# JanLohse/raw2film

Measured on AMD Instinct MI355X. Metric: megapixels/sec full film pipeline (neg+print+grain+halation+MTF), 100MP frame, higher is better.
Workload: dtype f32 (pointwise stages, grain) + f64 (FFT stencils; the MTF's scratch images are complex64)

## Files before the change

raw2film_amd/csrc/r2f_front.hip:

```cpp
#include <algorithm>
#include <type_traits>

#include "r2f_launch.h"

#include "../../include/r2f.h"

#ifndef R2F_FRONT_LUT_BATCH
#define R2F_FRONT_LUT_BATCH 4
#endif

namespace r2f {

namespace {

struct V3 {
    float2v xy;
    float z;
};

__device__ __forceinline__ float2v splat(float v) { return (float2v){v, v}; }

__device__ __forceinline__ V3 texel(const void* base, unsigned off) {
    const float4 t = *reinterpret_cast<const float4*>(static_cast<const char*>(base) + off);
    return V3{(float2v){t.x, t.y}, t.z};
}

__device__ __forceinline__ uint32_t u8_of(float v) {
    return (uint32_t)__builtin_amdgcn_fmed3f(v * 255.0f, 0.0f, 255.0f);
}

struct Mat3Pairs {
    float2v c0, c1, c2;
    float r0, r1, r2;
};
__device__ __forceinline__ Mat3Pairs pairs_of(const Mat3& M) {
    float m[6];
#pragma unroll
    for (int i = 0; i < 6; ++i) m[i] = __uint_as_float(__builtin_amdgcn_readfirstlane(__float_as_uint(M.m[i])));
    return Mat3Pairs{(float2v){m[0], m[3]}, (float2v){m[1], m[4]}, (float2v){m[2], m[5]}, M.m[6], M.m[7], M.m[8]};
}
__device__ __forceinline__ V3 matrix3(const Mat3Pairs& M, float r, float g, float b) {
    V3 o;
    o.xy = __builtin_elementwise_fma(M.c2, splat(b), __builtin_elementwise_fma(M.c1, splat(g), M.c0 * splat(r)));
    o.z = fmaf(M.r2, b, fmaf(M.r1, g, M.r0 * r));
    return o;
}

__device__ __forceinline__ V3 texel_lds(const float4* base, unsigned off) {
    const float4 t = *reinterpret_cast<const float4*>(reinterpret_cast<const char*>(base) + off);
    return V3{(float2v){t.x, t.y}, t.z};
}

__device__ __forceinline__ V3 lut2d(const float4* tex, const int n, const V3 p) {
#pragma clang fp contract(off)
    const float S = (p.xy.x + p.xy.y) + p.z;
    const bool dark = S < 1e-12f;
    const float inv_sum = (float)(n - 1) / (dark ? 1.0f : S);
    const float2v rg = p.xy * splat(inv_sum);
    const float fr = floorf(rg.x), fg = floorf(rg.y);
    const int ri = clampi((int)fr, 0, n - 2), gi = clampi((int)fg, 0, n - 2);
    const float rf = rg.x - fr, gf = rg.y - fg;
    const float fsum = rf + gf;
    const bool lower = fsum <= 1.0f;
    const unsigned n16 = (unsigned)n << 4;
    const unsigned o0 = (unsigned)(ri * n + gi) << 4;
    const V3 rv = texel_lds(tex, o0 + n16);
    const V3 gv = texel_lds(tex, o0 + 16u);
    const V3 sv = texel_lds(tex, o0 + (lower ? 0u : n16 + 16u));
    const float wr = lower ? rf : 1.0f - gf;
    const float wg = lower ? gf : 1.0f - rf;
    const float ws = lower ? 1.0f - fsum : fsum - 1.0f;
    const float Se = dark ? 0.0f : S;
    V3 o;
    o.xy = __builtin_elementwise_fma(sv.xy, splat(ws), __builtin_elementwise_fma(gv.xy, splat(wg), rv.xy * splat(wr))) * splat(Se);
    o.z = fmaf(sv.z, ws, fmaf(gv.z, wg, rv.z * wr)) * Se;
    return o;
}

__device__ __forceinline__ void axis_nonneg(float x, float s, int n, int& lo, float& d) {
    const float t = x * s;
    const int i0 = (int)t;
    lo = min(i0, n - 2);
    d = i0 >= n - 1 ? 1.0f : fmaf(x, s, -(float)i0);
}

__device__ __forceinline__ V3 lut3d_tetra_nonneg(const float4* tex, const int n, const float s, const float r, const float g,
                                                 const float b) {
    int rl, gl, bl;
    float dr, dg, db;
    axis_nonneg(r, s, n, rl, dr);
    axis_nonneg(g, s, n, gl, dg);
    axis_nonneg(b, s, n, bl, db);
    const unsigned er = (unsigned)(n * n) << 4, eg = (unsigned)n << 4, eb = 16u;
    const unsigned o0 = (unsigned)((rl * n + gl) * n + bl) << 4;
    const bool c1 = dr >= dg, c2 = dg >= db, c3 = dr >= db, c4 = db >= dg, c5 = db >= dr;
    const unsigned e1 = c1 ? ((c2 || c3) ? er : eb) : (c4 ? eb : eg);
    const unsigned e12 = c1 ? (c2 ? er + eg : er + eb) : ((c4 || c5) ? eg + eb : eg + er);
    const float d1 = fmaxf(fmaxf(dr, dg), db), d3 = fminf(fminf(dr, dg), db), d2 = __builtin_amdgcn_fmed3f(dr, dg, db);
    const V3 c0 = texel(tex, o0);
    const V3 ca = texel(tex, o0 + e1);
    const V3 cb = texel(tex, o0 + e12);
    const V3 cz = texel(tex, o0 + (er + eg + eb));
    V3 o;
    o.xy = __builtin_elementwise_fma(splat(d3), cz.xy - cb.xy,
                                     __builtin_elementwise_fma(splat(d2), cb.xy - ca.xy, __builtin_elementwise_fma(splat(d1), ca.xy - c0.xy, c0.xy)));
    o.z = fmaf(d3, cz.z - cb.z, fmaf(d2, cb.z - ca.z, fmaf(d1, ca.z - c0.z, c0.z)));
    return o;
}

template <int LAYOUT, int UPTO, int BY, bool FIN = false>
__global__ __launch_bounds__(64 * BY) void front_fast_kernel(const FrontArgs a) {
    extern __shared__ __attribute__((aligned(16))) float4 smem4[];
    float4* lut_lds = smem4;
    float4* cells_lds = smem4 + a.lut2d.n * a.lut2d.n;
    {
        const int tid = threadIdx.y * 64 + threadIdx.x;
        const int nt = a.lut2d.n * a.lut2d.n;
        for (int i = tid; i < nt; i += 64 * BY) lut_lds[i] = a.lut2d.tex[i];
        if (UPTO >= R2F_UPTO_DENSITY || FIN) {
            const int nc = 3 * (a.curve.m - 1);
            for (int i = tid; i < nc; i += 64 * BY) cells_lds[i] = a.curve.cells[i];
        }
        __syncthreads();
    }
#ifndef R2F_FRONT_UNITS
#define R2F_FRONT_UNITS 1
#endif
    const bool track = UPTO == R2F_UPTO_EXPOSURE && a.track.blk != nullptr;
    const int W = a.W;
    const float* in = static_cast<const float*>(a.in);
    const float s3 = a.lut3d_scale * (float)(a.lut3d.n - 1);
    const long long plane = (long long)a.in_rows * W;
    const Mat3Pairs mat = pairs_of(a.mat);
    auto row_loop = [&](auto trk_tag) {
    constexpr int TRK = decltype(trk_tag)::value;
    const int groups = (a.y1 - a.y0 + BY - 1) / BY;
    constexpr bool UNITS = R2F_FRONT_UNITS && UPTO == R2F_UPTO_OUTPUT;
    const int units = groups * a.gx;
    const int g_begin = UNITS ? (int)((long long)blockIdx.x * units / gridDim.x)
                              : (TRK ? (int)((long long)blockIdx.y * groups / gridDim.y) : (int)blockIdx.y);
    const int g_end = UNITS ? (int)((long long)(blockIdx.x + 1) * units / gridDim.x)
                            : (TRK ? (int)((long long)(blockIdx.y + 1) * groups / gridDim.y) : groups);
    const int g_step = (UNITS || TRK) ? 1 : (int)gridDim.y;
    float p_lo = __builtin_inff(), p_hi = 0.f;
    int p_ty = -1, p_tx = 0;
    auto flush = [&]() {
        if (p_ty < 0) return;
        const float w_lo = wave_extreme<false>(p_lo), w_hi = wave_extreme<true>(p_hi);
        if (threadIdx.x == 63) merge_tile(a.track, p_ty << kRangeTileRowsLog2, p_tx, w_lo, w_hi);
        p_lo = __builtin_inff(), p_hi = 0.f;
    };
    for (int unit = g_begin; unit < g_end; unit += g_step) {
        const int grp = UNITS ? unit / a.gx : unit;
        const int col = UNITS ? unit - grp * a.gx : (int)blockIdx.x;
        const int x = (col * 64 + threadIdx.x) * 4;
        const int gy = a.y0 + grp * BY + threadIdx.y;
        if (gy >= a.y1) continue;
        if (TRK) {
            const int ty = gy >> kRangeTileRowsLog2;
            if (ty != p_ty || col != p_tx) {
                flush();
                p_ty = ty, p_tx = col;
            }
        }
        if (x >= W) continue;
        const long long irow = gy - a.in_gy0;
        float r[4], g[4], b[4];
        if (LAYOUT == R2F_LAYOUT_CHW) {
            const float4 v0 = *reinterpret_cast<const float4*>(in + irow * W + x);
            const float4 v1 = *reinterpret_cast<const float4*>(in + plane + irow * W + x);
            const float4 v2 = *reinterpret_cast<const float4*>(in + 2 * plane + irow * W + x);
            r[0] = v0.x, r[1] = v0.y, r[2] = v0.z, r[3] = v0.w;
            g[0] = v1.x, g[1] = v1.y, g[2] = v1.z, g[3] = v1.w;
            b[0] = v2.x, b[1] = v2.y, b[2] = v2.z, b[3] = v2.w;
        } else if (LAYOUT == R2F_LAYOUT_HWC3) {
            const float4* p4 = reinterpret_cast<const float4*>(in + (irow * W + x) * 3);
            const float4 v0 = p4[0], v1 = p4[1], v2 = p4[2];
            r[0] = v0.x, g[0] = v0.y, b[0] = v0.z;
            r[1] = v0.w, g[1] = v1.x, b[1] = v1.y;
            r[2] = v1.z, g[2] = v1.w, b[2] = v2.x;
            r[3] = v2.y, g[3] = v2.z, b[3] = v2.w;
        } else {
            const float4* p4 = reinterpret_cast<const float4*>(in + (irow * W + x) * 4);
#pragma unroll
            for (int q = 0; q < 4; ++q) {
                const float4 v = p4[q];
                r[q] = v.x, g[q] = v.y, b[q] = v.z;
            }
        }
#pragma unroll
        for (int q = 0; q < 4; ++q) {
            V3 p = a.use_matrix ? matrix3(mat, r[q], g[q], b[q]) : V3{(float2v){r[q], g[q]}, b[q]};
            p = lut2d(lut_lds, a.lut2d.n, p);
            if (UPTO == R2F_UPTO_EXPOSURE) {
                r[q] = p.xy.x, g[q] = p.xy.y, b[q] = p.z;
                if (TRK == 1) {
                    p_lo = __builtin_isunordered(r[q], g[q]) ? -__builtin_inff() : fminf(fminf(p_lo, r[q]), g[q]);
                    p_hi = fmaxf(fmaxf(p_hi, fabsf(r[q])), fabsf(g[q]));
                } else if (TRK == 2) {
                    if (a.track_mask & 1) p_lo = range_min(p_lo, r[q]), p_hi = fmaxf(p_hi, fabsf(r[q]));
                    if (a.track_mask & 2) p_lo = range_min(p_lo, g[q]), p_hi = fmaxf(p_hi, fabsf(g[q]));
                    if (a.track_mask & 4) p_lo = range_min(p_lo, b[q]), p_hi = fmaxf(p_hi, fabsf(b[q]));
                }
                if (FIN) {
                    if (a.finish_mask & 1) r[q] = curve_eval_at((const float4*)cells_lds, a.curve, 0, log10_fast(a.finish_w[0] * r[q], a.log_eps));
                    if (a.finish_mask & 2) g[q] = curve_eval_at((const float4*)cells_lds, a.curve, 1, log10_fast(a.finish_w[1] * g[q], a.log_eps));
                    if (a.finish_mask & 4) b[q] = curve_eval_at((const float4*)cells_lds, a.curve, 2, log10_fast(a.finish_w[2] * b[q], a.log_eps));
                }
                continue;
            }
            float v3[3] = {log10_fast(p.xy.x, a.log_eps), log10_fast(p.xy.y, a.log_eps), log10_fast(p.z, a.log_eps)};
            curve_eval_batch<3, 3>((const float4*)cells_lds, a.curve, 0, v3);
            if (UPTO == R2F_UPTO_DENSITY) {
                r[q] = v3[0], g[q] = v3[1], b[q] = v3[2];
                continue;
            }
            if (R2F_FRONT_LUT_BATCH > 1) {
                r[q] = v3[0], g[q] = v3[1], b[q] = v3[2];
                continue;
            }
            if (__builtin_amdgcn_ballot_w64(fminf(fminf(v3[0], v3[1]), v3[2]) < 0.0f) == 0) {
                p = lut3d_tetra_nonneg(a.lut3d.tex, a.lut3d.n, s3, v3[0], v3[1], v3[2]);
                r[q] = p.xy.x, g[q] = p.xy.y, b[q] = p.z;
            } else {
                apply_lut3d_tetra(a.lut3d, s3, v3[0], v3[1], v3[2]);
                r[q] = v3[0], g[q] = v3[1], b[q] = v3[2];
            }
        }
        if (UPTO == R2F_UPTO_OUTPUT && R2F_FRONT_LUT_BATCH > 1) {
            constexpr int NB = R2F_FRONT_LUT_BATCH > 1 ? R2F_FRONT_LUT_BATCH : 2;
#pragma unroll
            for (int q0 = 0; q0 < 4; q0 += NB) {
                float rn[NB], gn[NB], bn[NB], lo = 0.f;
#pragma unroll
                for (int k = 0; k < NB; ++k) {
                    rn[k] = r[q0 + k], gn[k] = g[q0 + k], bn[k] = b[q0 + k];
                    lo = fminf(lo, fminf(fminf(rn[k], gn[k]), bn[k]));
                }
                if (__builtin_amdgcn_ballot_w64(lo < 0.0f) == 0) {
                    apply_lut3d_tetra_nonneg_batch<NB>(a.lut3d, s3, rn, gn, bn);
                } else {
#pragma unroll
                    for (int k = 0; k < NB; ++k) apply_lut3d_tetra(a.lut3d, s3, rn[k], gn[k], bn[k]);
                }
#pragma unroll
                for (int k = 0; k < NB; ++k) r[q0 + k] = rn[k], g[q0 + k] = gn[k], b[q0 + k] = bn[k];
            }
        }
        if (UPTO != R2F_UPTO_OUTPUT) {
            float* d0 = a.dst.data + (long long)(gy - a.dst.gy0) * W + x;
            float* f0 = FIN ? a.finish_dst.data + (long long)(gy - a.finish_dst.gy0) * W + x : d0;
            const long long fs = FIN ? a.finish_dst.plane_stride : 0;
            *reinterpret_cast<float4*>((FIN && (a.finish_mask & 1)) ? f0 : d0) = make_float4(r[0], r[1], r[2], r[3]);
            *reinterpret_cast<float4*>((FIN && (a.finish_mask & 2)) ? f0 + fs : d0 + a.dst.plane_stride) = make_float4(g[0], g[1], g[2], g[3]);
            *reinterpret_cast<float4*>((FIN && (a.finish_mask & 4)) ? f0 + 2 * fs : d0 + 2 * a.dst.plane_stride) =
                make_float4(b[0], b[1], b[2], b[3]);
            continue;
        }
        const long long obase = ((long long)(gy - a.out_gy0) * W + x) * 3;
        if (a.out_f32) {
            float4* o4 = reinterpret_cast<float4*>(a.out_f32 + obase);
            o4[0] = make_float4(r[0], g[0], b[0], r[1]);
            o4[1] = make_float4(g[1], b[1], r[2], g[2]);
            o4[2] = make_float4(b[2], r[3], g[3], b[3]);
        }
        if (a.out_u8) {
            uint32_t* o32 = reinterpret_cast<uint32_t*>(a.out_u8 + obase);
            o32[0] = u8_of(r[0]) | (u8_of(g[0]) << 8) | (u8_of(b[0]) << 16) | (u8_of(r[1]) << 24);
            o32[1] = u8_of(g[1]) | (u8_of(b[1]) << 8) | (u8_of(r[2]) << 16) | (u8_of(g[2]) << 24);
            o32[2] = u8_of(b[2]) | (u8_of(r[3]) << 8) | (u8_of(g[3]) << 16) | (u8_of(b[3]) << 24);
        }
    }
    if (TRK) {
        __shared__ int wg_ty[BY], wg_tx[BY];
        __shared__ float wg_lo[BY], wg_hi[BY];
        const float w_lo = wave_extreme<false>(p_lo), w_hi = wave_extreme<true>(p_hi);
        if (threadIdx.x == 63) wg_ty[threadIdx.y] = p_ty, wg_tx[threadIdx.y] = p_tx, wg_lo[threadIdx.y] = w_lo, wg_hi[threadIdx.y] = w_hi;
        __syncthreads();
        if (threadIdx.y == 0 && threadIdx.x == 0) {
            for (int i = 0; i < BY; ++i) {
                const int ty = wg_ty[i], tx = wg_tx[i];
                if (ty < 0) continue;
                float lo = wg_lo[i], hi = wg_hi[i];
                for (int j = i + 1; j < BY; ++j)
                    if (wg_ty[j] == ty && wg_tx[j] == tx) lo = fminf(lo, wg_lo[j]), hi = fmaxf(hi, wg_hi[j]), wg_ty[j] = -1;
                merge_tile(a.track, ty << kRangeTileRowsLog2, tx, lo, hi);
            }
        }
    }
    };
    if (!track)
        row_loop(std::integral_constant<int, 0>{});
    else if (a.track_mask == 3)
        row_loop(std::integral_constant<int, 1>{});
    else
        row_loop(std::integral_constant<int, 2>{});
}

size_t fast_lds_bytes(const FrontArgs& a) {
    const size_t lut = (size_t)a.lut2d.n * a.lut2d.n * sizeof(float4);
    const size_t cells = (a.upto >= R2F_UPTO_DENSITY || a.finish_mask) ? (size_t)3 * (a.curve.m > 1 ? a.curve.m - 1 : 0) * sizeof(float4) : 0;
    return lut + cells;
}

}

bool front_fast_eligible(const FrontArgs& a) {
    if (a.out_u16) return false;
    if (!a.vec || a.lut2d.n < 2 || (long long)a.W * 16 >= (1ll << 31) || fast_lds_bytes(a) > 144 * 1024) return false;
    if ((a.upto >= R2F_UPTO_DENSITY || a.finish_mask) && !(a.curve.near && a.curve.m >= 2)) return false;
    if (a.upto == R2F_UPTO_OUTPUT && !(a.lut3d_mode == 0 && a.lut3d.n >= 2 && a.lut3d.n <= 256)) return false;
    return true;
}

template <int UPTO, int BY, bool FIN = false>
static void launch_fast(const FrontArgs& a, hipStream_t s) {
    const int quads = (a.W + 3) / 4, gx = (quads + 63) / 64;
    const int row_groups = (a.y1 - a.y0 + BY - 1) / BY;
    const size_t lds = fast_lds_bytes(a);
    const int per_cu = lds > 80 * 1024 ? 1 : (BY == 16 ? 2 : (lds > 53 * 1024 ? 2 : 3));
    int gy = per_cu * 256 / gx;
    gy = gy > row_groups ? row_groups : (gy < 1 ? 1 : gy);
    dim3 grid(gx, gy);
    const dim3 block(64, BY);
    FrontArgs b = a;
    b.gx = gx;
    if (R2F_FRONT_UNITS && UPTO == R2F_UPTO_OUTPUT) {
        const long long units = (long long)gx * row_groups;
        grid = dim3((unsigned)std::min<long long>((long long)per_cu * 256, units));
    }
    switch (a.in_layout) {
        case R2F_LAYOUT_CHW: launch_k((front_fast_kernel<R2F_LAYOUT_CHW, UPTO, BY, FIN>), grid, block, lds, s, b); break;
        case R2F_LAYOUT_HWC3: launch_k((front_fast_kernel<R2F_LAYOUT_HWC3, UPTO, BY, FIN>), grid, block, lds, s, b); break;
        default: launch_k((front_fast_kernel<R2F_LAYOUT_HWC4, UPTO, BY, FIN>), grid, block, lds, s, b); break;
    }
}

hipError_t launch_front_fast(const FrontArgs& a, hipStream_t s) {
    const bool big = fast_lds_bytes(a) > 80 * 1024;
    if (a.upto == R2F_UPTO_EXPOSURE && a.finish_mask)
        big ? launch_fast<R2F_UPTO_EXPOSURE, 16, true>(a, s) : launch_fast<R2F_UPTO_EXPOSURE, 8, true>(a, s);
    else if (a.upto == R2F_UPTO_EXPOSURE)
        big ? launch_fast<R2F_UPTO_EXPOSURE, 16>(a, s) : launch_fast<R2F_UPTO_EXPOSURE, 8>(a, s);
    else if (a.upto == R2F_UPTO_DENSITY)
        big ? launch_fast<R2F_UPTO_DENSITY, 16>(a, s) : launch_fast<R2F_UPTO_DENSITY, 8>(a, s);
    else
        big ? launch_fast<R2F_UPTO_OUTPUT, 16>(a, s) : launch_fast<R2F_UPTO_OUTPUT, 8>(a, s);
    return take_launch_status();
}

hipError_t front_fast_init_attributes() {
#define R2F_FAST_ATTR(L, U, B)                                                                                             \
    {                                                                                                                     \
        hipError_t e = hipFuncSetAttribute(reinterpret_cast<const void*>(front_fast_kernel<L, U, B>),                     \
                                           hipFuncAttributeMaxDynamicSharedMemorySize, 144 * 1024);                       \
        if (e != hipSuccess) return e;                                                                                    \
        if (U == R2F_UPTO_EXPOSURE) {                                                                                     \
            e = hipFuncSetAttribute(reinterpret_cast<const void*>(front_fast_kernel<L, U, B, true>),                      \
                                    hipFuncAttributeMaxDynamicSharedMemorySize, 144 * 1024);                              \
            if (e != hipSuccess) return e;                                                                                \
        }                                                                                                                 \
    }
#define R2F_FAST_ATTR3(U, B) R2F_FAST_ATTR(R2F_LAYOUT_HWC3, U, B) R2F_FAST_ATTR(R2F_LAYOUT_HWC4, U, B) R2F_FAST_ATTR(R2F_LAYOUT_CHW, U, B)
    R2F_FAST_ATTR3(R2F_UPTO_EXPOSURE, 8)
    R2F_FAST_ATTR3(R2F_UPTO_EXPOSURE, 16)
    R2F_FAST_ATTR3(R2F_UPTO_DENSITY, 8)
    R2F_FAST_ATTR3(R2F_UPTO_DENSITY, 16)
    R2F_FAST_ATTR3(R2F_UPTO_OUTPUT, 8)
    R2F_FAST_ATTR3(R2F_UPTO_OUTPUT, 16)
#undef R2F_FAST_ATTR3
#undef R2F_FAST_ATTR
    return hipSuccess;
}

}
```

Before: 21610.

## Software-pipeline input loads across row units in front kernel

Restructures the front-stage row loop so that the next unit's input pixels are prefetched into registers while the current unit is computed. Depending on stage, the prefetch is issued early or after the LUT work, and asm barriers keep the loads from being sunk. It also inlines a specialized finish-curve evaluation with hoisted curve constants, and clamps x to W-4 instead of skipping out-of-range lanes. It adds experiment macros (R2F_FRONT_EXP) that replace loads or computation with constants for probing, all off by default. The cost is higher register pressure, which can lower occupancy.

```diff
diff --git a/raw2film_amd/csrc/r2f_front.hip b/raw2film_amd/csrc/r2f_front.hip
--- a/raw2film_amd/csrc/r2f_front.hip
+++ b/raw2film_amd/csrc/r2f_front.hip
@@ -7,6 +7,13 @@
 
 #ifndef R2F_FRONT_LUT_BATCH
 #define R2F_FRONT_LUT_BATCH 4
+#endif
+
+#ifndef R2F_FRONT_PIPE
+#define R2F_FRONT_PIPE 7
+#endif
+#ifndef R2F_FRONT_EXP
+#define R2F_FRONT_EXP 0
 #endif
 
 namespace r2f {
@@ -63,10 +70,14 @@
     const float fsum = rf + gf;
     const bool lower = fsum <= 1.0f;
     const unsigned n16 = (unsigned)n << 4;
-    const unsigned o0 = (unsigned)(ri * n + gi) << 4;
-    const V3 rv = texel_lds(tex, o0 + n16);
-    const V3 gv = texel_lds(tex, o0 + 16u);
-    const V3 sv = texel_lds(tex, o0 + (lower ? 0u : n16 + 16u));
+    unsigned o0 = (unsigned)(ri * n + gi) << 4;
+    if (R2F_FRONT_EXP & 4) {
+        asm volatile("" ::"v"(o0));
+        o0 = 0;
+    }
+    const V3 rv = (R2F_FRONT_EXP & 4) ? V3{(float2v){0.5f, 0.4f}, 0.3f} : texel_lds(tex, o0 + n16);
+    const V3 gv = (R2F_FRONT_EXP & 4) ? V3{(float2v){0.6f, 0.3f}, 0.2f} : texel_lds(tex, o0 + 16u);
+    const V3 sv = (R2F_FRONT_EXP & 4) ? V3{(float2v){0.4f, 0.5f}, 0.4f} : texel_lds(tex, o0 + (lower ? 0u : n16 + 16u));
     const float wr = lower ? rf : 1.0f - gf;
     const float wg = lower ? gf : 1.0f - rf;
     const float ws = lower ? 1.0f - fsum : fsum - 1.0f;
@@ -150,12 +161,85 @@
         if (threadIdx.x == 63) merge_tile(a.track, p_ty << kRangeTileRowsLog2, p_tx, w_lo, w_hi);
         p_lo = __builtin_inff(), p_hi = 0.f;
     };
-    for (int unit = g_begin; unit < g_end; unit += g_step) {
+    constexpr bool PIPE = ((R2F_FRONT_PIPE) >> UPTO) & 1;
+    constexpr int NV = LAYOUT == R2F_LAYOUT_HWC4 ? 4 : 3;
+    const int wave_row = __builtin_amdgcn_readfirstlane(threadIdx.y);
+    auto locate = [&](int unit, int& col, int& gy, int& x) {
         const int grp = UNITS ? unit / a.gx : unit;
-        const int col = UNITS ? unit - grp * a.gx : (int)blockIdx.x;
-        const int x = (col * 64 + threadIdx.x) * 4;
-        const int gy = a.y0 + grp * BY + threadIdx.y;
-        if (gy >= a.y1) continue;
+        col = UNITS ? unit - grp * a.gx : (int)blockIdx.x;
+        x = min((col * 64 + (int)threadIdx.x) * 4, W - 4);
+        gy = a.y0 + grp * BY + wave_row;
+    };
+    auto fetch = [&](int gy, int x, float4(&v)[NV]) {
+        const long long irow = gy - a.in_gy0;
+        if (R2F_FRONT_EXP & 1) {
+            const float t = 0.05f + 1e-4f * (float)((x + 7 * gy) & 1023);
+#pragma unroll
+            for (int i = 0; i < NV; ++i) v[i] = make_float4(t, 2.f * t, 0.5f * t + 0.01f * i, 3.f * t);
+        } else if (LAYOUT == R2F_LAYOUT_CHW) {
+            v[0] = *reinterpret_cast<const float4*>(in + irow * W + x);
+            v[1] = *reinterpret_cast<const float4*>(in + plane + irow * W + x);
+            v[2] = *reinterpret_cast<const float4*>(in + 2 * plane + irow * W + x);
+        } else {
+            const float4* p4 = reinterpret_cast<const float4*>(in + (irow * W + x) * (LAYOUT == R2F_LAYOUT_HWC3 ? 3 : 4));
+#pragma unroll
+            for (int i = 0; i < NV; ++i) v[i] = p4[i];
+        }
+    };
+    auto fin_log = [&](float e) {
+        float l = log10_fast(e, a.log_eps);
+        if (R2F_FRONT_EXP & 4) {
+            asm volatile("" ::"v"(l));
+            l = -1.0f;
+        }
+        return l;
+    };
+    const int c_last = a.curve.m - 2;
+    const float c_x0 = a.curve.x0, c_x1 = a.curve.x1, c_inv = a.curve.inv_step;
+    const float c_first[3] = {a.curve.f_first[0], a.curve.f_first[1], a.curve.f_first[2]};
+    const float c_last_v[3] = {a.curve.f_last[0], a.curve.f_last[1], a.curve.f_last[2]};
+    auto fin_curve = [&](int ch, float e) {
+        const float x = fin_log(e);
+        const float4* cells = (const float4*)cells_lds + ch * (a.curve.m - 1);
+        const int i = clampi((int)((x - c_x0) * c_inv), 0, c_last);
+        float4 c = cells[i];
+        const int adj = (x < c.x && i > 0) ? -1 : ((x >= c.y && i < c_last) ? 1 : 0);
+        c = cells[i + adj];
+        const float v = fmaf(c.w, x - c.x, c.z);
+        return !(x > c_x0) ? c_first[ch] : (x >= c_x1 ? c_last_v[ch] : v);
+    };
+    float4 nv[NV];
+#pragma unroll
+    for (int i = 0; i < NV; ++i) nv[i] = make_float4(0.f, 0.f, 0.f, 0.f);
+    int n_col = 0, n_gy = 0, n_x = 0;
+    constexpr bool LATE = PIPE && UPTO == R2F_UPTO_OUTPUT;
+    auto prefetch = [&](int unit) {
+        locate(unit, n_col, n_gy, n_x);
+        fetch(min(n_gy, a.y1 - 1), n_x, nv);
+    };
+    auto settle = [&]() {
+        if (PIPE && !LATE && !(R2F_FRONT_EXP & 1)) {
+#pragma unroll
+            for (int i = 0; i < NV; ++i) asm volatile("" : "+v"(nv[i].x), "+v"(nv[i].y), "+v"(nv[i].z), "+v"(nv[i].w)::"memory");
+        }
+    };
+    if (PIPE && g_begin < g_end) prefetch(g_begin);
+    settle();
+    auto unit_body = [&](const int unit) {
+        int col, gy, x;
+        float4 v[NV];
+        if (PIPE) {
+            col = n_col, gy = n_gy, x = n_x;
+#pragma unroll
+            for (int i = 0; i < NV; ++i) v[i] = nv[i];
+            if (!LATE) prefetch(unit + g_step);
+        } else {
+            locate(unit, col, gy, x);
+        }
+        if (!LATE && gy >= a.y1) {
+            settle();
+            return;
+        }
         if (TRK) {
             const int ty = gy >> kRangeTileRowsLog2;
             if (ty != p_ty || col != p_tx) {
@@ -163,30 +247,20 @@
                 p_ty = ty, p_tx = col;
             }
         }
-        if (x >= W) continue;
-        const long long irow = gy - a.in_gy0;
+        if (!PIPE) fetch(gy, x, v);
         float r[4], g[4], b[4];
         if (LAYOUT == R2F_LAYOUT_CHW) {
-            const float4 v0 = *reinterpret_cast<const float4*>(in + irow * W + x);
-            const float4 v1 = *reinterpret_cast<const float4*>(in + plane + irow * W + x);
-            const float4 v2 = *reinterpret_cast<const float4*>(in + 2 * plane + irow * W + x);
-            r[0] = v0.x, r[1] = v0.y, r[2] = v0.z, r[3] = v0.w;
-            g[0] = v1.x, g[1] = v1.y, g[2] = v1.z, g[3] = v1.w;
-            b[0] = v2.x, b[1] = v2.y, b[2] = v2.z, b[3] = v2.w;
+            r[0] = v[0].x, r[1] = v[0].y, r[2] = v[0].z, r[3] = v[0].w;
+            g[0] = v[1].x, g[1] = v[1].y, g[2] = v[1].z, g[3] = v[1].w;
+            b[0] = v[2].x, b[1] = v[2].y, b[2] = v[2].z, b[3] = v[2].w;
         } else if (LAYOUT == R2F_LAYOUT_HWC3) {
-            const float4* p4 = reinterpret_cast<const float4*>(in + (irow * W + x) * 3);
-            const float4 v0 = p4[0], v1 = p4[1], v2 = p4[2];
-            r[0] = v0.x, g[0] = v0.y, b[0] = v0.z;
-            r[1] = v0.w, g[1] = v1.x, b[1] = v1.y;
-            r[2] = v1.z, g[2] = v1.w, b[2] = v2.x;
-            r[3] = v2.y, g[3] = v2.z, b[3] = v2.w;
+            r[0] = v[0].x, g[0] = v[0].y, b[0] = v[0].z;
+            r[1] = v[0].w, g[1] = v[1].x, b[1] = v[1].y;
+            r[2] = v[1].z, g[2] = v[1].w, b[2] = v[2].x;
+            r[3] = v[2].y, g[3] = v[2].z, b[3] = v[2].w;
         } else {
-            const float4* p4 = reinterpret_cast<const float4*>(in + (irow * W + x) * 4);
-#pragma unroll
-            for (int q = 0; q < 4; ++q) {
-                const float4 v = p4[q];
-                r[q] = v.x, g[q] = v.y, b[q] = v.z;
-            }
+#pragma unroll
+            for (int q = 0; q < 4; ++q) r[q] = v[q].x, g[q] = v[q].y, b[q] = v[q].z;
         }
 #pragma unroll
         for (int q = 0; q < 4; ++q) {
@@ -203,9 +277,9 @@
                     if (a.track_mask & 4) p_lo = range_min(p_lo, b[q]), p_hi = fmaxf(p_hi, fabsf(b[q]));
                 }
                 if (FIN) {
-                    if (a.finish_mask & 1) r[q] = curve_eval_at((const float4*)cells_lds, a.curve, 0, log10_fast(a.finish_w[0] * r[q], a.log_eps));
-                    if (a.finish_mask & 2) g[q] = curve_eval_at((const float4*)cells_lds, a.curve, 1, log10_fast(a.finish_w[1] * g[q], a.log_eps));
-                    if (a.finish_mask & 4) b[q] = curve_eval_at((const float4*)cells_lds, a.curve, 2, log10_fast(a.finish_w[2] * b[q], a.log_eps));
+                    if (a.finish_mask & 1) r[q] = fin_curve(0, a.finish_w[0] * r[q]);
+                    if (a.finish_mask & 2) g[q] = fin_curve(1, a.finish_w[1] * g[q]);
+                    if (a.finish_mask & 4) b[q] = fin_curve(2, a.finish_w[2] * b[q]);
                 }
                 continue;
             }
@@ -246,6 +320,14 @@
 #pragma unroll
                 for (int k = 0; k < NB; ++k) r[q0 + k] = rn[k], g[q0 + k] = gn[k], b[q0 + k] = bn[k];
             }
+        }
+        if (LATE) {
+            prefetch(unit + g_step);
+            if (gy >= a.y1) return;
+        }
+        if ((R2F_FRONT_EXP & 2) && (r[0] + g[1]) + b[2] != 1.2345e30f) {
+            settle();
+            return;
         }
         if (UPTO != R2F_UPTO_OUTPUT) {
             float* d0 = a.dst.data + (long long)(gy - a.dst.gy0) * W + x;
@@ -255,7 +337,8 @@
             *reinterpret_cast<float4*>((FIN && (a.finish_mask & 2)) ? f0 + fs : d0 + a.dst.plane_stride) = make_float4(g[0], g[1], g[2], g[3]);
             *reinterpret_cast<float4*>((FIN && (a.finish_mask & 4)) ? f0 + 2 * fs : d0 + 2 * a.dst.plane_stride) =
                 make_float4(b[0], b[1], b[2], b[3]);
-            continue;
+            settle();
+            return;
         }
         const long long obase = ((long long)(gy - a.out_gy0) * W + x) * 3;
         if (a.out_f32) {
@@ -270,6 +353,9 @@
             o32[1] = u8_of(g[1]) | (u8_of(b[1]) << 8) | (u8_of(r[2]) << 16) | (u8_of(g[2]) << 24);
             o32[2] = u8_of(b[2]) | (u8_of(r[3]) << 8) | (u8_of(g[3]) << 16) | (u8_of(b[3]) << 24);
         }
+    };
+    for (int unit = g_begin; unit < g_end; unit += g_step) {
+        unit_body(unit);
     }
     if (TRK) {
         __shared__ int wg_ty[BY], wg_tx[BY];
```

New measurement: 21310. 0.986x the previous value.
